# SJCaldwell/NanoDiloco

Hardware: AMD Instinct MI355X
Metric: tokens/sec (whole node) Llama-150M, 8 DiLoCo workers H=100; bytes/outer-step (higher is better)
Workload: dtype bf16; 1 GPU; model=Llama-150M, global_batch=256, seq_len=1024, parallelism=diloco1, per_worker_batch=256, micro_batch=128, grad_accum=2, inner_steps_H=100, params=214983680

## Files before the change

### nanodiloco_amd/csrc/cross_entropy.hip

```cpp
#include "common.h"
#include <cstdio>
#include <cstdlib>

using namespace nd;

struct ZArgs {
  float coef;
  float* z_sum;
  float* row_z;
};
__device__ __forceinline__ const ZArgs& zarg(const ZArgs& z) { return z; }

__device__ __forceinline__ void z_commit(const ZArgs& z, int64_t row, bool valid, float lse) {
  if (z.row_z) z.row_z[row] = valid ? lse * lse : 0.f;
  else if (valid) atomicAdd(z.z_sum, lse * lse);
}

template <int NT>
__device__ __forceinline__ float block_max(float v, float* red) {
  v = wave_max(v);
  const int w = threadIdx.x >> 6, l = threadIdx.x & 63;
  __syncthreads();
  if (l == 0) red[w] = v;
  __syncthreads();
  float t = red[0];
#pragma unroll
  for (int i = 1; i < NT / 64; ++i) t = fmaxf(t, red[i]);
  return t;
}

template <int DT, int CH, class... ZA>
__global__ void __launch_bounds__(256) ce_reg_kernel(void* __restrict__ logits, const int64_t* __restrict__ targets,
                                                     float* __restrict__ loss_sum, const float* __restrict__ scale_p,
                                                     int V, int ignore, float* __restrict__ lse_out,
                                                     float* __restrict__ row_loss, ZA... z) {
  constexpr bool Z = sizeof...(ZA) > 0;
  __shared__ float red[8];
  const int64_t row = blockIdx.x;
  const int64_t base = row * (int64_t)V;
  const int64_t tgt = targets[row];
  const bool valid = tgt != ignore;
  float x[CH][8];
  float m = -INFINITY;
#pragma unroll
  for (int c = 0; c < CH; ++c) {
    const int col = (c * 256 + threadIdx.x) * 8;
    if (col < V) {
      Vec8<DT>::load(logits, base + col, x[c]);
#pragma unroll
      for (int j = 0; j < 8; ++j) m = fmaxf(m, x[c][j]);
    }
  }
  m = block_max<256>(m, red);
  float s = 0.f;
#pragma unroll
  for (int c = 0; c < CH; ++c) {
    const int col = (c * 256 + threadIdx.x) * 8;
    if (col < V) {
#pragma unroll
      for (int j = 0; j < 8; ++j) s += __expf(x[c][j] - m);
    }
  }
  __syncthreads();
  s = block_sum<256>(s, red);
  const float lse = m + __logf(s);
  const float sc = valid ? scale_p[0] : 0.f;
  float scg = sc;
  if constexpr (Z) scg = valid ? sc * fmaf(2.f * zarg(z...).coef, lse, 1.f) : 0.f;
  float picked = 0.f;
#pragma unroll
  for (int c = 0; c < CH; ++c) {
    const int col = (c * 256 + threadIdx.x) * 8;
    if (col < V) {
      float o[8];
#pragma unroll
      for (int j = 0; j < 8; ++j) {
        const bool hit = (int64_t)(col + j) == tgt;
        if (hit) picked = x[c][j];
        if constexpr (Z) o[j] = fmaf(__expf(x[c][j] - lse), scg, hit ? -sc : 0.f);
        else o[j] = (__expf(x[c][j] - lse) - (hit ? 1.f : 0.f)) * sc;
      }
      Vec8<DT>::store(logits, base + col, o);
    }
  }
  if (threadIdx.x == 0) {
    if (lse_out) lse_out[row] = lse;
  }
  __syncthreads();
  picked = block_sum<256>(picked, red);
  if (threadIdx.x == 0) {
    if (row_loss) row_loss[row] = valid ? lse - picked : 0.f;
    else if (valid) atomicAdd(loss_sum, lse - picked);
    if constexpr (Z) z_commit(zarg(z...), row, valid, lse);
  }
}


template <int CH, int QF = -1, class... ZA>
__global__ void __launch_bounds__(256) ce_bf16_kernel(bf16_t* __restrict__ logits, const int64_t* __restrict__ targets,
                                                      float* __restrict__ loss_sum, const float* __restrict__ scale_p,
                                                      int V, int ignore, float* __restrict__ lse_out,
                                                     float* __restrict__ row_loss, Fp8Out q8, ZA... z) {
  constexpr bool Z = sizeof...(ZA) > 0;
  constexpr float L2E = 1.4426950408889634f, LN2 = 0.6931471805599453f;
  __shared__ float red[8];
  const int64_t row = blockIdx.x;
  bf16_t* rp = logits + row * (int64_t)V;
  const int tgt = (int)targets[row];
  const bool valid = tgt != ignore;
  uint4 x[CH];
  float m = -INFINITY;
#pragma unroll
  for (int c = 0; c < CH; ++c) {
    const int col = (c * 256 + threadIdx.x) * 8;
    if (col < V) {
      x[c] = *reinterpret_cast<const uint4*>(rp + col);
      const uint32_t u[4] = {x[c].x, x[c].y, x[c].z, x[c].w};
#pragma unroll
      for (int j = 0; j < 4; ++j) m = fmaxf(m, fmaxf(lo_bf(u[j]), hi_bf(u[j])));
    }
  }
  m = block_max<256>(m, red);
  const float m2 = m * L2E;
#pragma unroll
  for (int c = 0; c < CH; ++c) asm volatile("" : "+v"(x[c].x), "+v"(x[c].y), "+v"(x[c].z), "+v"(x[c].w));
  float s = 0.f;
#pragma unroll
  for (int c = 0; c < CH; ++c) {
    const int col = (c * 256 + threadIdx.x) * 8;
    if (col < V) {
      const uint32_t u[4] = {x[c].x, x[c].y, x[c].z, x[c].w};
#pragma unroll
      for (int j = 0; j < 4; ++j)
        s += __builtin_amdgcn_exp2f(fmaf(lo_bf(u[j]), L2E, -m2)) + __builtin_amdgcn_exp2f(fmaf(hi_bf(u[j]), L2E, -m2));
    }
  }
  __syncthreads();
  s = block_sum<256>(s, red);
  const float lse2 = m2 + __log2f(s);
#pragma unroll
  for (int c = 0; c < CH; ++c) asm volatile("" : "+v"(x[c].x), "+v"(x[c].y), "+v"(x[c].z), "+v"(x[c].w));
  const float sc = valid ? scale_p[0] : 0.f;
  float scg = sc;
  if constexpr (Z) scg = valid ? sc * fmaf(2.f * zarg(z...).coef, lse2 * LN2, 1.f) : 0.f;
  const float qsc = QF >= 0 ? q8.scale[0] : 1.f;
  float qmax = 0.f;
  float picked = 0.f;
#pragma unroll
  for (int c = 0; c < CH; ++c) {
    const int col = (c * 256 + threadIdx.x) * 8;
    if (col < V) {
      const uint32_t u[4] = {x[c].x, x[c].y, x[c].z, x[c].w};
      float o[8];
#pragma unroll
      for (int j = 0; j < 4; ++j) {
        o[2 * j] = __builtin_amdgcn_exp2f(fmaf(lo_bf(u[j]), L2E, -lse2)) * scg;
        o[2 * j + 1] = __builtin_amdgcn_exp2f(fmaf(hi_bf(u[j]), L2E, -lse2)) * scg;
      }
      const unsigned d = (unsigned)(tgt - col);
      if (d < 8u) {
#pragma unroll
        for (int j = 0; j < 8; ++j)
          if ((unsigned)j == d) {
            picked = (j & 1) ? hi_bf(u[j >> 1]) : lo_bf(u[j >> 1]);
            o[j] -= sc;
          }
      }
      uint4 w;
      w.x = pack2(o[0], o[1]); w.y = pack2(o[2], o[3]); w.z = pack2(o[4], o[5]); w.w = pack2(o[6], o[7]);
      if constexpr (QF < 0) {
        *reinterpret_cast<uint4*>(rp + col) = w;
      } else {
        const float r[8] = {lo_bf(w.x), hi_bf(w.x), lo_bf(w.y), hi_bf(w.y), lo_bf(w.z), hi_bf(w.z), lo_bf(w.w), hi_bf(w.w)};
#pragma unroll
        for (int j = 0; j < 8; ++j) qmax = fmaxf(qmax, fabsf(r[j]));
        uint2 o8;
        o8.x = cvt4<QF>(r[0] * qsc, r[1] * qsc, r[2] * qsc, r[3] * qsc);
        o8.y = cvt4<QF>(r[4] * qsc, r[5] * qsc, r[6] * qsc, r[7] * qsc);
        *reinterpret_cast<uint2*>(q8.q + row * (int64_t)V + col) = o8;
      }
    }
  }
  if constexpr (QF >= 0) block_amax_commit<256>(qmax, q8.amax, q8.parts);
  const float lse = lse2 * LN2;
  if (threadIdx.x == 0 && lse_out) lse_out[row] = lse;
  __syncthreads();
  picked = block_sum<256>(picked, red);
  if (threadIdx.x == 0) {
    if (row_loss) row_loss[row] = valid ? lse - picked : 0.f;
    else if (valid) atomicAdd(loss_sum, lse - picked);
    if constexpr (Z) z_commit(zarg(z...), row, valid, lse);
  }
}

template <int DT, class... ZA>
__global__ void __launch_bounds__(256) ce_generic_kernel(void* __restrict__ logits, const int64_t* __restrict__ targets,
                                                         float* __restrict__ loss_sum, const float* __restrict__ scale_p,
                                                         int V, int ignore, float* __restrict__ lse_out,
                                                     float* __restrict__ row_loss, ZA... z) {
  constexpr bool Z = sizeof...(ZA) > 0;
  __shared__ float red[8];
  const int64_t row = blockIdx.x;
  const int64_t base = row * (int64_t)V;
  const int64_t tgt = targets[row];
  const bool valid = tgt != ignore;
  auto ld = [&](int j) -> float {
    if (DT == BF16) return bf2f(reinterpret_cast<const bf16_t*>(logits)[base + j]);
    return reinterpret_cast<const float*>(logits)[base + j];
  };
  float m = -INFINITY, s = 0.f;
  for (int j = threadIdx.x; j < V; j += 256) {
    const float v = ld(j);
    const float nm = fmaxf(m, v);
    s = s * __expf(m - nm) + __expf(v - nm);
    m = nm;
  }
  const float gm = block_max<256>(m, red);
  s = s * __expf(m - gm);
  __syncthreads();
  s = block_sum<256>(s, red);
  const float lse = gm + __logf(s);
  const float sc = valid ? scale_p[0] : 0.f;
  float scg = sc;
  if constexpr (Z) scg = valid ? sc * fmaf(2.f * zarg(z...).coef, lse, 1.f) : 0.f;
  float picked = 0.f;
  for (int j = threadIdx.x; j < V; j += 256) {
    const float v = ld(j);
    const bool hit = (int64_t)j == tgt;
    if (hit) picked = v;
    float o;
    if constexpr (Z) o = fmaf(__expf(v - lse), scg, hit ? -sc : 0.f);
    else o = (__expf(v - lse) - (hit ? 1.f : 0.f)) * sc;
    if (DT == BF16) reinterpret_cast<bf16_t*>(logits)[base + j] = f2bf(o);
    else reinterpret_cast<float*>(logits)[base + j] = o;
  }
  if (threadIdx.x == 0 && lse_out) lse_out[row] = lse;
  __syncthreads();
  picked = block_sum<256>(picked, red);
  if (threadIdx.x == 0) {
    if (row_loss) row_loss[row] = valid ? lse - picked : 0.f;
    else if (valid) atomicAdd(loss_sum, lse - picked);
    if constexpr (Z) z_commit(zarg(z...), row, valid, lse);
  }
}

static bool parse_ce_env() {
  const char* e = getenv("ND_CE");
  return e && e[0] == 'r';
}
static bool g_ce_reg = parse_ce_env();
namespace nd {
void ce_env_reload() { g_ce_reg = parse_ce_env(); }
int ce_env_describe(char* buf, int n) { return snprintf(buf, n > 0 ? n : 0, "ND_CE=%s", g_ce_reg ? "r" : "d"); }
}

ND_API int nd_ce_fwd_bwd(void* logits, int dt, const int64_t* targets, float* loss_sum, const float* scale,
                         int64_t n, int V, int ignore, float* lse_out, float* row_loss, float ,
                         hipStream_t s) {
  if (n <= 0) return 0;
  dim3 g((unsigned)n), b(256);
  if (V % 8 == 0 && V <= 256 * 8 * 16) {
    if (V <= 256 * 8 * 4) {
      if (dt == BF16) hipLaunchKernelGGL((ce_reg_kernel<BF16, 4>), g, b, 0, s, logits, targets, loss_sum, scale, V, ignore, lse_out, row_loss);
      else hipLaunchKernelGGL((ce_reg_kernel<F32, 4>), g, b, 0, s, logits, targets, loss_sum, scale, V, ignore, lse_out, row_loss);
    } else {
      if (dt == BF16 && !g_ce_reg)
        hipLaunchKernelGGL((ce_bf16_kernel<16>), g, b, 0, s, (bf16_t*)logits, targets, loss_sum, scale, V, ignore, lse_out, row_loss,
                           Fp8Out{nullptr, nullptr, nullptr, 1, 0});
      else if (dt == BF16) hipLaunchKernelGGL((ce_reg_kernel<BF16, 16>), g, b, 0, s, logits, targets, loss_sum, scale, V, ignore, lse_out, row_loss);
      else hipLaunchKernelGGL((ce_reg_kernel<F32, 16>), g, b, 0, s, logits, targets, loss_sum, scale, V, ignore, lse_out, row_loss);
    }
  } else {
    if (dt == BF16) hipLaunchKernelGGL(ce_generic_kernel<BF16>, g, b, 0, s, logits, targets, loss_sum, scale, V, ignore, lse_out, row_loss);
    else hipLaunchKernelGGL(ce_generic_kernel<F32>, g, b, 0, s, logits, targets, loss_sum, scale, V, ignore, lse_out, row_loss);
  }
  ND_LAUNCH_CHECK();
}

ND_API int nd_ce_fwd_bwd_q8(void* logits, int dt, const int64_t* targets, float* loss_sum, const float* scale,
                            int64_t n, int V, int ignore, float* lse_out, float* row_loss, void* q, const float* qscale,
                            float* amax, int parts, int fmt, hipStream_t s) {
  if (n <= 0) return 0;
  if (dt != BF16 || V % 8 != 0 || V <= 256 * 8 * 4 || V > 256 * 8 * 16 || g_ce_reg || !q || !qscale || !amax ||
      parts < 1 || (fmt != 0 && fmt != 1))
    return (int)hipErrorInvalidValue;
  const Fp8Out q8{(uint8_t*)q, qscale, amax, parts, fmt};
  dim3 g((unsigned)n), b(256);
  if (fmt == 0)
    hipLaunchKernelGGL((ce_bf16_kernel<16, 0>), g, b, 0, s, (bf16_t*)logits, targets, loss_sum, scale, V, ignore, lse_out,
                       row_loss, q8);
  else
    hipLaunchKernelGGL((ce_bf16_kernel<16, 1>), g, b, 0, s, (bf16_t*)logits, targets, loss_sum, scale, V, ignore, lse_out,
                       row_loss, q8);
  ND_LAUNCH_CHECK();
}

static bool z_args_ok(const float* z_sum, const float* row_z, float z_coef) {
  return (z_sum || row_z) && z_coef >= 0.f && z_coef <= 3.0e38f;
}

ND_API int nd_ce_z_fwd_bwd(void* logits, int dt, const int64_t* targets, float* loss_sum, float* z_sum,
                           const float* scale, int64_t n, int V, int ignore, float* lse_out, float* row_loss,
                           float* row_z, float z_coef, hipStream_t s) {
  if (!z_args_ok(z_sum, row_z, z_coef)) return (int)hipErrorInvalidValue;
  if (n <= 0) return 0;
  const ZArgs z{z_coef, z_sum, row_z};
  dim3 g((unsigned)n), b(256);
  if (V % 8 == 0 && V <= 256 * 8 * 16) {
    if (V <= 256 * 8 * 4) {
      if (dt == BF16) hipLaunchKernelGGL((ce_reg_kernel<BF16, 4, ZArgs>), g, b, 0, s, logits, targets, loss_sum, scale, V, ignore, lse_out, row_loss, z);
      else hipLaunchKernelGGL((ce_reg_kernel<F32, 4, ZArgs>), g, b, 0, s, logits, targets, loss_sum, scale, V, ignore, lse_out, row_loss, z);
    } else {
      if (dt == BF16 && !g_ce_reg)
        hipLaunchKernelGGL((ce_bf16_kernel<16, -1, ZArgs>), g, b, 0, s, (bf16_t*)logits, targets, loss_sum, scale, V, ignore, lse_out, row_loss,
                           Fp8Out{nullptr, nullptr, nullptr, 1, 0}, z);
      else if (dt == BF16) hipLaunchKernelGGL((ce_reg_kernel<BF16, 16, ZArgs>), g, b, 0, s, logits, targets, loss_sum, scale, V, ignore, lse_out, row_loss, z);
      else hipLaunchKernelGGL((ce_reg_kernel<F32, 16, ZArgs>), g, b, 0, s, logits, targets, loss_sum, scale, V, ignore, lse_out, row_loss, z);
    }
  } else {
    if (dt == BF16) hipLaunchKernelGGL((ce_generic_kernel<BF16, ZArgs>), g, b, 0, s, logits, targets, loss_sum, scale, V, ignore, lse_out, row_loss, z);
    else hipLaunchKernelGGL((ce_generic_kernel<F32, ZArgs>), g, b, 0, s, logits, targets, loss_sum, scale, V, ignore, lse_out, row_loss, z);
  }
  ND_LAUNCH_CHECK();
}

ND_API int nd_ce_z_fwd_bwd_q8(void* logits, int dt, const int64_t* targets, float* loss_sum, float* z_sum,
                              const float* scale, int64_t n, int V, int ignore, float* lse_out, float* row_loss,
                              float* row_z, float z_coef, void* q, const float* qscale, float* amax, int parts, int fmt,
                              hipStream_t s) {
  if (!z_args_ok(z_sum, row_z, z_coef)) return (int)hipErrorInvalidValue;
  if (n <= 0) return 0;
  if (dt != BF16 || V % 8 != 0 || V <= 256 * 8 * 4 || V > 256 * 8 * 16 || g_ce_reg || !q || !qscale || !amax ||
      parts < 1 || (fmt != 0 && fmt != 1))
    return (int)hipErrorInvalidValue;
  const Fp8Out q8{(uint8_t*)q, qscale, amax, parts, fmt};
  const ZArgs z{z_coef, z_sum, row_z};
  dim3 g((unsigned)n), b(256);
  if (fmt == 0)
    hipLaunchKernelGGL((ce_bf16_kernel<16, 0, ZArgs>), g, b, 0, s, (bf16_t*)logits, targets, loss_sum, scale, V, ignore, lse_out,
                       row_loss, q8, z);
  else
    hipLaunchKernelGGL((ce_bf16_kernel<16, 1, ZArgs>), g, b, 0, s, (bf16_t*)logits, targets, loss_sum, scale, V, ignore, lse_out,
                       row_loss, q8, z);
  ND_LAUNCH_CHECK();
}
```

### nanodiloco_amd/csrc/embedding.hip

```cpp
#include "common.h"

using namespace nd;

__device__ __forceinline__ void put4(float* out, int64_t i, float4 v) { *reinterpret_cast<float4*>(out + i) = v; }
__device__ __forceinline__ void put4(bf16_t* out, int64_t i, float4 v) {
  *reinterpret_cast<uint2*>(out + i) = make_uint2(pack2(v.x, v.y), pack2(v.z, v.w));
}
__device__ __forceinline__ float4 get4(const float* p, int64_t i) { return *reinterpret_cast<const float4*>(p + i); }
__device__ __forceinline__ float4 get4(const bf16_t* p, int64_t i) {
  const uint2 u = *reinterpret_cast<const uint2*>(p + i);
  return make_float4(lo_bf(u.x), hi_bf(u.x), lo_bf(u.y), hi_bf(u.y));
}
__device__ __forceinline__ float get1(const float* p, int64_t i) { return p[i]; }
__device__ __forceinline__ float get1(const bf16_t* p, int64_t i) { return bf2f(p[i]); }

template <typename OT>
__global__ void __launch_bounds__(256) embed_fwd_kernel(const int64_t* __restrict__ ids, const float* __restrict__ W,
                                                        OT* __restrict__ out, int64_t n, int d, int V) {
  const int lane = threadIdx.x & 63;
  const int64_t wave = (int64_t)blockIdx.x * 4 + (threadIdx.x >> 6);
  for (int64_t r = wave; r < n; r += (int64_t)gridDim.x * 4) {
    const int64_t id = ids[r];
    const bool ok = id >= 0 && id < V;
    for (int c = lane * 4; c < d; c += 256) {
      float4 v = ok ? *reinterpret_cast<const float4*>(W + id * d + c) : make_float4(0.f, 0.f, 0.f, 0.f);
      put4(out, r * d + c, v);
    }
  }
}

template <typename DT>
__global__ void __launch_bounds__(256) embed_bwd_kernel(const int64_t* __restrict__ ids, const DT* __restrict__ dy,
                                                        float* __restrict__ gW, int64_t n, int d, int V) {
  const int lane = threadIdx.x & 63;
  const int64_t wave = (int64_t)blockIdx.x * 4 + (threadIdx.x >> 6);
  for (int64_t r = wave; r < n; r += (int64_t)gridDim.x * 4) {
    const int64_t id = ids[r];
    if (id < 0 || id >= V) continue;
    for (int c = lane; c < d; c += 64) atomicAdd(gW + id * d + c, get1(dy, r * d + c));
  }
}

constexpr int kEmbChunk = 64;

template <typename DT>
__global__ void __launch_bounds__(256) embed_bwd_sorted_chunks_kernel(const int64_t* __restrict__ sid,
                                                                      const int64_t* __restrict__ perm,
                                                                      const DT* __restrict__ dy,
                                                                      float* __restrict__ gW, float* __restrict__ head,
                                                                      float* __restrict__ tail, int64_t n, int d, int V) {
  const int lane = threadIdx.x & 63;
  const int64_t nchunks = (n + kEmbChunk - 1) / kEmbChunk;
  for (int64_t c = (int64_t)blockIdx.x * 4 + (threadIdx.x >> 6); c < nchunks; c += (int64_t)gridDim.x * 4) {
    const int64_t cs = c * kEmbChunk, ce = cs + kEmbChunk < n ? cs + kEmbChunk : n;
    for (int64_t j = cs; j < ce;) {
      const int64_t id = sid[j];
      int64_t e = j + 1;
      while (e < ce && sid[e] == id) ++e;
      if (id >= 0 && id < V) {
        const bool cont_in = j == cs && cs > 0 && sid[cs - 1] == id;
        const bool cont_out = e == ce && ce < n && sid[ce] == id;
        float* dst = cont_in ? head + c * d : cont_out ? tail + c * d : gW + id * d;
        for (int col = lane * 4; col < d; col += 256) {
          float4 acc = make_float4(0.f, 0.f, 0.f, 0.f);
          for (int64_t k = j; k < e; ++k) {
            const float4 v = get4(dy, perm[k] * d + col);
            acc.x += v.x; acc.y += v.y; acc.z += v.z; acc.w += v.w;
          }
          float4* g = reinterpret_cast<float4*>(dst + col);
          if (!cont_in && !cont_out) {
            const float4 o = *g;
            acc.x += o.x; acc.y += o.y; acc.z += o.z; acc.w += o.w;
          }
          *g = acc;
        }
      }
      j = e;
    }
  }
}

__global__ void __launch_bounds__(256) embed_bwd_sorted_join_kernel(const int64_t* __restrict__ sid,
                                                                    float* __restrict__ gW,
                                                                    const float* __restrict__ head,
                                                                    const float* __restrict__ tail, int64_t n, int d,
                                                                    int V) {
  const int lane = threadIdx.x & 63;
  const int64_t nchunks = (n + kEmbChunk - 1) / kEmbChunk;
  for (int64_t c = (int64_t)blockIdx.x * 4 + (threadIdx.x >> 6); c < nchunks; c += (int64_t)gridDim.x * 4) {
    const int64_t cs = c * kEmbChunk, ce = cs + kEmbChunk < n ? cs + kEmbChunk : n;
    const int64_t id = sid[ce - 1];
    if (ce >= n || sid[ce] != id || id < 0 || id >= V) continue;
    if (sid[cs] == id && cs > 0 && sid[cs - 1] == id) continue;
    for (int col = lane * 4; col < d; col += 256) {
      float4 acc = *reinterpret_cast<const float4*>(tail + c * d + col);
      for (int64_t k = c + 1; k < nchunks; ++k) {
        const float4 v = *reinterpret_cast<const float4*>(head + k * d + col);
        acc.x += v.x; acc.y += v.y; acc.z += v.z; acc.w += v.w;
        const int64_t ke = (k + 1) * kEmbChunk;
        if (ke >= n || sid[ke] != id) break;
      }
      float4* g = reinterpret_cast<float4*>(gW + id * d + col);
      const float4 o = *g;
      acc.x += o.x; acc.y += o.y; acc.z += o.z; acc.w += o.w;
      *g = acc;
    }
  }
}

ND_API int nd_embedding_bwd_sorted(const int64_t* sid, const int64_t* perm, const void* dy, int ddt, float* gW,
                                   float* ws, int64_t n, int d, int V, hipStream_t s) {
  if (d % 4) return (int)hipErrorInvalidValue;
  if (n <= 0) return 0;
  const int64_t nchunks = (n + kEmbChunk - 1) / kEmbChunk;
  float* head = ws;
  float* tail = ws + nchunks * d;
  int64_t blocks = (nchunks + 3) / 4;
  if (blocks > 8192) blocks = 8192;
  if (ddt == F32)
    hipLaunchKernelGGL(embed_bwd_sorted_chunks_kernel<float>, dim3((unsigned)blocks), dim3(256), 0, s, sid, perm,
                       (const float*)dy, gW, head, tail, n, d, V);
  else if (ddt == BF16)
    hipLaunchKernelGGL(embed_bwd_sorted_chunks_kernel<bf16_t>, dim3((unsigned)blocks), dim3(256), 0, s, sid, perm,
                       (const bf16_t*)dy, gW, head, tail, n, d, V);
  else
    return (int)hipErrorInvalidValue;
  if (hipError_t e = hipGetLastError(); e != hipSuccess) return (int)e;
  hipLaunchKernelGGL(embed_bwd_sorted_join_kernel, dim3((unsigned)blocks), dim3(256), 0, s, sid, gW, head, tail, n, d,
                     V);
  ND_LAUNCH_CHECK();
}

ND_API int nd_embedding_fwd(const int64_t* ids, const float* W, void* out, int odt, int64_t n, int d, int V,
                            hipStream_t s) {
  if (d % 4) return (int)hipErrorInvalidValue;
  int64_t blocks = (n + 3) / 4;
  if (blocks > 8192) blocks = 8192;
  if (odt == F32)
    hipLaunchKernelGGL(embed_fwd_kernel<float>, dim3((unsigned)blocks), dim3(256), 0, s, ids, W, (float*)out, n, d, V);
  else if (odt == BF16)
    hipLaunchKernelGGL(embed_fwd_kernel<bf16_t>, dim3((unsigned)blocks), dim3(256), 0, s, ids, W, (bf16_t*)out, n, d,
                       V);
  else
    return (int)hipErrorInvalidValue;
  ND_LAUNCH_CHECK();
}

ND_API int nd_embedding_bwd(const int64_t* ids, const void* dy, int ddt, float* gW, int64_t n, int d, int V,
                            hipStream_t s) {
  int64_t blocks = (n + 3) / 4;
  if (blocks > 8192) blocks = 8192;
  if (ddt == F32)
    hipLaunchKernelGGL(embed_bwd_kernel<float>, dim3((unsigned)blocks), dim3(256), 0, s, ids, (const float*)dy, gW, n,
                       d, V);
  else if (ddt == BF16)
    hipLaunchKernelGGL(embed_bwd_kernel<bf16_t>, dim3((unsigned)blocks), dim3(256), 0, s, ids, (const bf16_t*)dy, gW,
                       n, d, V);
  else
    return (int)hipErrorInvalidValue;
  ND_LAUNCH_CHECK();
}
```

### nanodiloco_amd/ops/_ext.py

```python
from __future__ import annotations

import ctypes
import os
import threading
from typing import Optional

import torch

_HERE = os.path.dirname(os.path.abspath(__file__))
LIB_DIR = os.path.join(os.path.dirname(_HERE), "_lib")
LIB_PATH = os.path.join(LIB_DIR, "libnd_kernels.so")
LIB_PATH = os.environ.get("ND_KERNELS_LIB") or LIB_PATH

_lib = None
_lock = threading.Lock()
_backend = os.environ.get("NANODILOCO_OPS", "auto")


class ExtensionMissing(RuntimeError):
    pass


def set_backend(name: str):
    global _backend
    if name not in ("auto", "hip", "torch"):
        raise ValueError(name)
    _backend = name


def get_backend() -> str:
    return _backend


def lib() -> ctypes.CDLL:
    global _lib
    if _lib is None:
        with _lock:
            if _lib is None:
                if not os.path.exists(LIB_PATH):
                    raise ExtensionMissing(
                        f"HIP kernel library not found at {LIB_PATH}. Build it with "
                        f"`python -m nanodiloco_amd.csrc.build` (or __graft_entry__.build()).")
                raw = ctypes.CDLL(LIB_PATH, mode=ctypes.RTLD_GLOBAL)
                _declare(raw)
                _lib = _StrictLib(raw)
    return _lib


def load_library(path: str) -> "_StrictLib":
    raw = ctypes.CDLL(path, mode=ctypes.RTLD_LOCAL)
    _declare(raw)
    return _StrictLib(raw)


class using:

    def __init__(self, other):
        self.other = other

    def __enter__(self):
        global _lib
        self.prev = lib()
        _lib = self.other
        return self.other

    def __exit__(self, *exc):
        global _lib
        _lib = self.prev
        return False


def available() -> bool:
    try:
        lib()
        return True
    except (ExtensionMissing, OSError):
        return False


def use_hip(t: torch.Tensor) -> bool:
    if not t.is_cuda:
        if _backend == "hip":
            raise RuntimeError("backend 'hip' requested for a CPU tensor")
        return False
    if _backend == "torch":
        return False
    lib()
    return True


def stream_ptr(device: torch.device = None) -> int:
    return torch.cuda.current_stream(device).cuda_stream


def ptr(t: Optional[torch.Tensor]) -> int:
    return 0 if t is None else t.data_ptr()


DT_F32, DT_BF16 = 0, 1


def dtcode(t: torch.Tensor) -> int:
    if t.dtype == torch.float32:
        return DT_F32
    if t.dtype == torch.bfloat16:
        return DT_BF16
    raise TypeError(f"unsupported dtype {t.dtype}")


def _declare(L: ctypes.CDLL):
    P, I, F, L64, D = ctypes.c_void_p, ctypes.c_int, ctypes.c_float, ctypes.c_int64, ctypes.c_double
    sigs = {
        "nd_version": [],
        "nd_env_reload": [],
        "nd_env_describe": [P, I],
        "nd_rmsnorm_fwd": [P, I, P, I, P, P, I, P, P, L64, I, F, P],
        "nd_rmsnorm_bwd": [P, I, P, I, P, P, P, P, I, P, L64, I, P, P],
        "nd_colsum_add": [P, P, I, I, P],
        "nd_rmsnorm_fwd_q": [P, I, P, I, P, P, I, P, P, L64, I, F, P, P, P, I, I, P],
        "nd_rmsnorm_bwd_q": [P, I, P, I, P, P, P, P, I, P, L64, I, P, P, P, P, I, I, P],
        "nd_transpose_bf16": [P, P, I, I, L64, L64, P],
        "nd_rope_inplace": [P, I, P, P, L64, I, I, I, I, I, I, P],
        "nd_attn_fwd": [P, P, P, P, P, I, I, I, I, I, L64, L64, P, P, F, P],
        "nd_attn_fwd_ks": [P, P, P, P, P, I, I, I, I, I, L64, L64, P, P, F, P, P],
        "nd_attn_bwd_ks": [P, P, P, P, P, P, P, P, P, P, I, I, I, I, I, L64, L64, P, P, F, I, P, P],
        "nd_attn_bwd_fused_ks": [P, P, P, P, P, P, P, P, P, P, I, I, I, I, I, L64, L64, P, P, F, I, P, P],
        "nd_attn_fwd_doc": [P, P, P, P, P, I, I, I, I, I, L64, L64, P, P, F, P, P, P],
        "nd_attn_bwd_fused_doc": [P, P, P, P, P, P, P, P, P, P, I, I, I, I, I, L64, L64, P, P, F, I, P, P, P],
        "nd_attn_bwd_pre": [P, P, P, I, I, I, L64, L64, P],
        "nd_attn_bwd": [P, P, P, P, P, P, P, P, P, P, I, I, I, I, I, L64, L64, P, P, F, I, P],
        "nd_attn_bwd_fused": [P, P, P, P, P, P, P, P, P, P, I, I, I, I, I, L64, L64, P, P, F, I, P],
        "nd_attn_decode": [P, P, P, P, P, P, P, P, P, P, I, I, I, I, I, L64, F, P],
        "nd_attn_decode_split": [],
        "nd_swiglu_fwd": [P, P, I, L64, I, P],
        "nd_swiglu_bwd": [P, P, P, I, L64, I, P],
        "nd_swiglu_fwd_q": [P, P, L64, I, P, P, P, I, I, P],
        "nd_swiglu_bwd_q": [P, P, P, L64, I, P, P, P, I, I, P],
        "nd_ce_fwd_bwd": [P, I, P, P, P, L64, I, I, P, P, F, P],
        "nd_ce_fwd_bwd_q8": [P, I, P, P, P, L64, I, I, P, P, P, P, P, I, I, P],
        "nd_ce_z_fwd_bwd": [P, I, P, P, P, P, L64, I, I, P, P, P, F, P],
        "nd_ce_z_fwd_bwd_q8": [P, I, P, P, P, P, L64, I, I, P, P, P, F, P, P, P, I, I, P],
        "nd_ce_loss": [P, I, P, L64, I, I, P, P, P, P],
        "nd_embedding_fwd": [P, P, P, I, L64, I, I, P],
        "nd_embedding_bwd": [P, P, I, P, L64, I, I, P],
        "nd_embedding_bwd_sorted": [P, P, P, I, P, P, L64, I, I, P],
        "nd_sumsq_partial": [P, L64, P, I, P],
        "nd_adamw_step": [P, P, P, P, P, I, L64, P, I, F, D, D, F, F, F, F, F, P, I, P, P],
        "nd_pseudograd": [P, P, P, I, L64, P],
        "nd_outer_nesterov": [P, P, P, I, P, P, I, L64, F, F, F, I, P, P, P],
        "nd_axpby": [P, P, L64, F, F, P],
        "nd_frag_pseudograd": [P, P, P, I, L64, P, I, P],
        "nd_frag_outer_mix": [P, P, P, I, P, P, I, P, I, L64, F, F, F, I, F, P],
        "nd_adamw_step_spans": [P, P, P, P, P, I, P, I, L64, P, I, F, D, D, F, F, F, F, F, P, I, P, P],
        "nd_pseudograd_q": [P, P, L64, P, L64, L64, I, P],
        "nd_qreduce": [P, I, L64, I, P, P],
        "nd_pseudograd_q_ef": [P, P, P, L64, P, L64, L64, I, P],
        "nd_qreduce_ef": [P, I, L64, I, P, P, P],
        "nd_outer_nesterov_q": [P, P, P, I, L64, P, P, I, L64, F, F, F, I, P],
        "nd_pseudograd_topk": [P, P, P, L64, P, I, I, P],
        "nd_outer_nesterov_topk": [P, P, P, I, I, I, P, P, I, L64, F, F, F, I, P],
        "nd_lowrank_project": [P, P, P, P, P, P, P, I, P, P, I, I, L64, L64, L64, P],
        "nd_lowrank_orthonormalize": [P, P, P, I, I, L64, P],
        "nd_lowrank_backproject": [P, P, P, P, P, I, I, L64, L64, L64, P],
        "nd_outer_nesterov_lowrank": [P, P, P, P, P, P, P, P, P, I, P, P, P, I, P, P, I, I, L64, L64, L64, F, F, F, I, P],
        "nd_fp8_cast":[P, I, L64, P, P, I, P, I, P],
        "nd_fp8_cast_t": [P, I, I, I, L64, P, P, P, I, P, I, P],
        "nd_gemm_pp": [P, P, P, I, I, I, L64, L64, L64, P],
        "nd_gemm_pp_rope": [P, P, P, I, I, I, L64, L64, L64, P, P, I, I, I, P],
        "nd_gemm_pp_swiglu": [P, P, P, P, I, I, I, L64, L64, L64, L64, P],
        "nd_gemm_pp_dswiglu": [P, P, P, P, I, I, I, L64, L64, L64, L64, P],
        "nd_gemm_pp_f8": [P, P, P, I, I, I, L64, L64, L64, P, P, I, P],
        "nd_gemm_pp_rope_f8": [P, P, P, I, I, I, L64, L64, L64, P, P, P, P, I, I, I, P],
        "nd_gemm_pp_swiglu_f8": [P, P, P, P, I, I, I, L64, L64, L64, L64, P, P, P],
        "nd_gemm_pp_dswiglu_f8": [P, P, P, P, I, I, I, L64, L64, L64, L64, P, P, I, P],
        "nd_gemm_pp_set_group_m": [I],
        "nd_mlp_coef_set": [I],
        "nd_probe_tr8": [P, P, P, P],
        "nd_gemm_pp_swiglu_f8q": [P, P, P, P, I, I, I, L64, L64, L64, L64, P, P, P, P, I, P],
        "nd_gemm_pp_dswiglu_f8q": [P, P, P, P, I, I, I, L64, L64, L64, L64, P, P, I, P, P, I, P],
        "nd_wgrad_f8": [P, P, P, P, I, I, I, L64, L64, L64, P, P, I, P],
        "nd_gemm_pp_set_variant": [I],
        "nd_gemm_w128": [P, P, P, I, I, I, L64, L64, L64, P],
        "nd_gemm_w128_set": [I, I, I],
        "nd_gemm_w128_set_ablation": [I],
        "nd_gemm_w128_set_vb": [I],
        "nd_wgrad_splits": [I, I, I],
        "nd_wgrad_f8_splits": [I, I, I],
        "nd_wgrad_force_splits": [I],
        "nd_wgrad": [P, P, P, P, I, I, I, L64, L64, L64, P],
        "nd_wgrad2_splits": [I, I, I, I, I],
        "nd_wgrad2": [P, P, P, P, I, I, L64, L64, L64, P, P, P, P, I, I, L64, L64, L64, I, P],
    }
    for name, argtypes in sigs.items():
        fn = getattr(L, name, None)
        if fn is None:
            continue
        fn.argtypes = argtypes
        fn.restype = ctypes.c_int


class _StrictLib:

    def __init__(self, raw):
        self._raw = raw
        self._fns = {}

    def __getattr__(self, name):
        f = self._fns.get(name)
        if f is None:
            fn = getattr(self._raw, name)
            n = len(fn.argtypes) if fn.argtypes is not None else None

            def f(*args, _fn=fn, _n=n, _name=name):
                if _n is not None and len(args) != _n:
                    raise TypeError(f"{_name}: expected {_n} arguments, got {len(args)}")
                return _fn(*args)

            self._fns[name] = f
        return f


def check(err: int, what: str):
    if err != 0:
        raise RuntimeError(f"{what} failed with hipError {err}")
```

### nanodiloco_amd/ops/embedding.py

```python
from __future__ import annotations

import torch

from . import _ext
from .determinism import deterministic


class EmbeddingFn(torch.autograd.Function):
    @staticmethod
    def forward(ctx, ids, w, gw, anchor, out_dtype=None):
        ids = ids.reshape(-1)
        ctx.save_for_backward(ids)
        ctx.gw = gw
        ctx.vocab = w.shape[0]
        odt = out_dtype or w.dtype
        if _ext.use_hip(w) and w.dtype == torch.float32:
            n, d = ids.numel(), w.shape[1]
            out = torch.empty(n, d, dtype=odt, device=w.device)
            _ext.check(_ext.lib().nd_embedding_fwd(_ext.ptr(ids), _ext.ptr(w), _ext.ptr(out), _ext.dtcode(out), n, d,
                                                   w.shape[0], _ext.stream_ptr(w.device)), "nd_embedding_fwd")
            ctx.hip = True
            return out
        ctx.hip = False
        return w.index_select(0, ids).to(odt)

    @staticmethod
    def backward(ctx, dy):
        (ids,) = ctx.saved_tensors
        if ctx.gw is not None:
            dy = dy.contiguous()
            if ctx.hip:
                n, d = dy.shape
                if deterministic():
                    perm = torch.argsort(ids, stable=True)
                    sid = ids.index_select(0, perm).contiguous()
                    ws = sorted_bwd_workspace(n, d, dy.device)
                    _ext.check(_ext.lib().nd_embedding_bwd_sorted(
                        _ext.ptr(sid), _ext.ptr(perm), _ext.ptr(dy), _ext.dtcode(dy), _ext.ptr(ctx.gw), _ext.ptr(ws),
                        n, d, ctx.vocab, _ext.stream_ptr(dy.device)), "nd_embedding_bwd_sorted")
                else:
                    _ext.check(_ext.lib().nd_embedding_bwd(_ext.ptr(ids), _ext.ptr(dy), _ext.dtcode(dy),
                                                           _ext.ptr(ctx.gw), n, d, ctx.vocab,
                                                           _ext.stream_ptr(dy.device)), "nd_embedding_bwd")
            else:
                ctx.gw.index_add_(0, ids, dy.float())
        from .linear import join_wgrad
        join_wgrad(dy.device if dy.is_cuda else None)
        return None, None, None, None, None


_ANCHORS = {}

SORTED_CHUNK = 64


def sorted_bwd_workspace(n, d, device):
    return torch.empty(2 * ((n + SORTED_CHUNK - 1) // SORTED_CHUNK) * d, dtype=torch.float32, device=device)


def _anchor(device):
    a = _ANCHORS.get(device)
    if a is None:
        a = torch.zeros(0, device=device, requires_grad=True)
        _ANCHORS[device] = a
    return a


def embedding(ids, w, gw, out_dtype=None):
    return EmbeddingFn.apply(ids, w, gw, _anchor(w.device), out_dtype)
```

Measured before the change: 829,400 tokens/s.

## Use buffer loads/stores with non-temporal hints in CE kernel; always use sorted embedding bwd

The bf16 cross-entropy kernel now reads and writes logits through AMD buffer resource loads and stores with a non-temporal cache hint. Hardware bounds checking replaces the per-column branch, and out-of-range lanes are filled with -inf. Separately, the atomic embedding backward path is deleted, so the sorted deterministic path (argsort plus segmented reduce) always runs. The sorted path adds argsort cost when determinism is not requested, but it removes atomic contention on the embedding gradient.

```diff
diff --git a/nanodiloco_amd/csrc/cross_entropy.hip b/nanodiloco_amd/csrc/cross_entropy.hip
--- a/nanodiloco_amd/csrc/cross_entropy.hip
+++ b/nanodiloco_amd/csrc/cross_entropy.hip
@@ -1,4 +1,4 @@
-#include "common.h"
+#include "lds_dma.h"
 #include <cstdio>
 #include <cstdlib>
 
@@ -96,6 +96,9 @@
 }
 
 
+constexpr int kNt = 2;
+typedef uint32_t u32x4_t __attribute__((ext_vector_type(4)));
+typedef uint32_t u32x2_t __attribute__((ext_vector_type(2)));
 template <int CH, int QF = -1, class... ZA>
 __global__ void __launch_bounds__(256) ce_bf16_kernel(bf16_t* __restrict__ logits, const int64_t* __restrict__ targets,
                                                       float* __restrict__ loss_sum, const float* __restrict__ scale_p,
@@ -108,13 +111,17 @@
   bf16_t* rp = logits + row * (int64_t)V;
   const int tgt = (int)targets[row];
   const bool valid = tgt != ignore;
+  const __amdgpu_buffer_rsrc_t rr = rsrc(rp, (uint32_t)V * 2u);
+  const uint32_t vo = threadIdx.x * 16u;
   uint4 x[CH];
+#pragma unroll
+  for (int c = 0; c < CH; ++c)
+    x[c] = __builtin_bit_cast(uint4, __builtin_amdgcn_raw_buffer_load_b128(rr, vo, c * 4096, kNt));
   float m = -INFINITY;
 #pragma unroll
   for (int c = 0; c < CH; ++c) {
-    const int col = (c * 256 + threadIdx.x) * 8;
-    if (col < V) {
-      x[c] = *reinterpret_cast<const uint4*>(rp + col);
+    if (c * 2048 < V) {
+      if ((c * 256 + (int)threadIdx.x) * 8 >= V) x[c] = make_uint4(0xff80ff80u, 0xff80ff80u, 0xff80ff80u, 0xff80ff80u);
       const uint32_t u[4] = {x[c].x, x[c].y, x[c].z, x[c].w};
 #pragma unroll
       for (int j = 0; j < 4; ++j) m = fmaxf(m, fmaxf(lo_bf(u[j]), hi_bf(u[j])));
@@ -127,8 +134,7 @@
   float s = 0.f;
 #pragma unroll
   for (int c = 0; c < CH; ++c) {
-    const int col = (c * 256 + threadIdx.x) * 8;
-    if (col < V) {
+    if (c * 2048 < V) {
       const uint32_t u[4] = {x[c].x, x[c].y, x[c].z, x[c].w};
 #pragma unroll
       for (int j = 0; j < 4; ++j)
@@ -144,12 +150,13 @@
   float scg = sc;
   if constexpr (Z) scg = valid ? sc * fmaf(2.f * zarg(z...).coef, lse2 * LN2, 1.f) : 0.f;
   const float qsc = QF >= 0 ? q8.scale[0] : 1.f;
+  const __amdgpu_buffer_rsrc_t qr = rsrc(QF >= 0 ? q8.q + row * (int64_t)V : nullptr, QF >= 0 ? (uint32_t)V : 0u);
   float qmax = 0.f;
   float picked = 0.f;
 #pragma unroll
   for (int c = 0; c < CH; ++c) {
     const int col = (c * 256 + threadIdx.x) * 8;
-    if (col < V) {
+    if (c * 2048 < V) {
       const uint32_t u[4] = {x[c].x, x[c].y, x[c].z, x[c].w};
       float o[8];
 #pragma unroll
@@ -169,7 +176,7 @@
       uint4 w;
       w.x = pack2(o[0], o[1]); w.y = pack2(o[2], o[3]); w.z = pack2(o[4], o[5]); w.w = pack2(o[6], o[7]);
       if constexpr (QF < 0) {
-        *reinterpret_cast<uint4*>(rp + col) = w;
+        __builtin_amdgcn_raw_buffer_store_b128(__builtin_bit_cast(u32x4_t, w), rr, vo, c * 4096, kNt);
       } else {
         const float r[8] = {lo_bf(w.x), hi_bf(w.x), lo_bf(w.y), hi_bf(w.y), lo_bf(w.z), hi_bf(w.z), lo_bf(w.w), hi_bf(w.w)};
 #pragma unroll
@@ -177,7 +184,7 @@
         uint2 o8;
         o8.x = cvt4<QF>(r[0] * qsc, r[1] * qsc, r[2] * qsc, r[3] * qsc);
         o8.y = cvt4<QF>(r[4] * qsc, r[5] * qsc, r[6] * qsc, r[7] * qsc);
-        *reinterpret_cast<uint2*>(q8.q + row * (int64_t)V + col) = o8;
+        __builtin_amdgcn_raw_buffer_store_b64(__builtin_bit_cast(u32x2_t, o8), qr, vo >> 1, c * 2048, kNt);
       }
     }
   }
diff --git a/nanodiloco_amd/csrc/embedding.hip b/nanodiloco_amd/csrc/embedding.hip
--- a/nanodiloco_amd/csrc/embedding.hip
+++ b/nanodiloco_amd/csrc/embedding.hip
@@ -11,8 +11,6 @@
   const uint2 u = *reinterpret_cast<const uint2*>(p + i);
   return make_float4(lo_bf(u.x), hi_bf(u.x), lo_bf(u.y), hi_bf(u.y));
 }
-__device__ __forceinline__ float get1(const float* p, int64_t i) { return p[i]; }
-__device__ __forceinline__ float get1(const bf16_t* p, int64_t i) { return bf2f(p[i]); }
 
 template <typename OT>
 __global__ void __launch_bounds__(256) embed_fwd_kernel(const int64_t* __restrict__ ids, const float* __restrict__ W,
@@ -26,18 +24,6 @@
       float4 v = ok ? *reinterpret_cast<const float4*>(W + id * d + c) : make_float4(0.f, 0.f, 0.f, 0.f);
       put4(out, r * d + c, v);
     }
-  }
-}
-
-template <typename DT>
-__global__ void __launch_bounds__(256) embed_bwd_kernel(const int64_t* __restrict__ ids, const DT* __restrict__ dy,
-                                                        float* __restrict__ gW, int64_t n, int d, int V) {
-  const int lane = threadIdx.x & 63;
-  const int64_t wave = (int64_t)blockIdx.x * 4 + (threadIdx.x >> 6);
-  for (int64_t r = wave; r < n; r += (int64_t)gridDim.x * 4) {
-    const int64_t id = ids[r];
-    if (id < 0 || id >= V) continue;
-    for (int c = lane; c < d; c += 64) atomicAdd(gW + id * d + c, get1(dy, r * d + c));
   }
 }
 
@@ -145,18 +131,3 @@
     return (int)hipErrorInvalidValue;
   ND_LAUNCH_CHECK();
 }
-
-ND_API int nd_embedding_bwd(const int64_t* ids, const void* dy, int ddt, float* gW, int64_t n, int d, int V,
-                            hipStream_t s) {
-  int64_t blocks = (n + 3) / 4;
-  if (blocks > 8192) blocks = 8192;
-  if (ddt == F32)
-    hipLaunchKernelGGL(embed_bwd_kernel<float>, dim3((unsigned)blocks), dim3(256), 0, s, ids, (const float*)dy, gW, n,
-                       d, V);
-  else if (ddt == BF16)
-    hipLaunchKernelGGL(embed_bwd_kernel<bf16_t>, dim3((unsigned)blocks), dim3(256), 0, s, ids, (const bf16_t*)dy, gW,
-                       n, d, V);
-  else
-    return (int)hipErrorInvalidValue;
-  ND_LAUNCH_CHECK();
-}
diff --git a/nanodiloco_amd/ops/_ext.py b/nanodiloco_amd/ops/_ext.py
--- a/nanodiloco_amd/ops/_ext.py
+++ b/nanodiloco_amd/ops/_ext.py
@@ -142,7 +142,6 @@
         "nd_ce_z_fwd_bwd_q8": [P, I, P, P, P, P, L64, I, I, P, P, P, F, P, P, P, I, I, P],
         "nd_ce_loss": [P, I, P, L64, I, I, P, P, P, P],
         "nd_embedding_fwd": [P, P, P, I, L64, I, I, P],
-        "nd_embedding_bwd": [P, P, I, P, L64, I, I, P],
         "nd_embedding_bwd_sorted": [P, P, P, I, P, P, L64, I, I, P],
         "nd_sumsq_partial": [P, L64, P, I, P],
         "nd_adamw_step": [P, P, P, P, P, I, L64, P, I, F, D, D, F, F, F, F, F, P, I, P, P],
diff --git a/nanodiloco_amd/ops/embedding.py b/nanodiloco_amd/ops/embedding.py
--- a/nanodiloco_amd/ops/embedding.py
+++ b/nanodiloco_amd/ops/embedding.py
@@ -3,7 +3,6 @@
 import torch
 
 from . import _ext
-from .determinism import deterministic
 
 
 class EmbeddingFn(torch.autograd.Function):
@@ -31,17 +30,12 @@
             dy = dy.contiguous()
             if ctx.hip:
                 n, d = dy.shape
-                if deterministic():
-                    perm = torch.argsort(ids, stable=True)
-                    sid = ids.index_select(0, perm).contiguous()
-                    ws = sorted_bwd_workspace(n, d, dy.device)
-                    _ext.check(_ext.lib().nd_embedding_bwd_sorted(
-                        _ext.ptr(sid), _ext.ptr(perm), _ext.ptr(dy), _ext.dtcode(dy), _ext.ptr(ctx.gw), _ext.ptr(ws),
-                        n, d, ctx.vocab, _ext.stream_ptr(dy.device)), "nd_embedding_bwd_sorted")
-                else:
-                    _ext.check(_ext.lib().nd_embedding_bwd(_ext.ptr(ids), _ext.ptr(dy), _ext.dtcode(dy),
-                                                           _ext.ptr(ctx.gw), n, d, ctx.vocab,
-                                                           _ext.stream_ptr(dy.device)), "nd_embedding_bwd")
+                perm = torch.argsort(ids, stable=True)
+                sid = ids.index_select(0, perm).contiguous()
+                ws = sorted_bwd_workspace(n, d, dy.device)
+                _ext.check(_ext.lib().nd_embedding_bwd_sorted(
+                    _ext.ptr(sid), _ext.ptr(perm), _ext.ptr(dy), _ext.dtcode(dy), _ext.ptr(ctx.gw), _ext.ptr(ws),
+                    n, d, ctx.vocab, _ext.stream_ptr(dy.device)), "nd_embedding_bwd_sorted")
             else:
                 ctx.gw.index_add_(0, ids, dy.float())
         from .linear import join_wgrad
```

After: 831,100 tokens/s (median of 6 runs). No clear change (+0.2%).
